# caishiqing/voice-tts

Hardware: AMD Instinct MI355X
Metric: audio_seconds_per_second (higher is better)
Workload: dtype bf16

## Files before the change

voice-tts_amd/csrc/gemm_x6.hip:

```cpp
#include "common.h"

namespace ixtts {

typedef float gx_f32x16 __attribute__((ext_vector_type(16)));
typedef __bf16 gx_bf16x8 __attribute__((ext_vector_type(8)));
typedef float gx_f32x4 __attribute__((ext_vector_type(4)));
typedef unsigned int gx_u32x4 __attribute__((ext_vector_type(4)));


__global__ void gemm_x6_pack_kernel(const float* __restrict__ w, uint4* __restrict__ out, int N, int K, int Npad) {
  const long total = (long)(K / 8) * Npad;
  for (long idx = blockIdx.x * (long)blockDim.x + threadIdx.x; idx < total; idx += (long)gridDim.x * blockDim.x) {
    const int n = (int)(idx % Npad);
    const int ko = (int)(idx / Npad);
    float v[8];
#pragma unroll
    for (int e = 0; e < 8; ++e) v[e] = n < N ? w[(long)n * K + ko * 8 + e] : 0.f;
    uint4 ph, pm, pl;
    split8_bf16x3(v, ph, pm, pl);
    const int g = ko >> 1, kh = ko & 1;
    uint4* base = out + ((long)g * 6) * Npad + n;
    base[(long)(0 * 2 + kh) * Npad] = ph;
    base[(long)(1 * 2 + kh) * Npad] = pm;
    base[(long)(2 * 2 + kh) * Npad] = pl;
  }
}

__global__ __launch_bounds__(256) void gemm_x6_split_kernel(const float* __restrict__ a, long lda, uint4* __restrict__ out, int M, int K, long Mpad) {
  __shared__ float tile[64][65];
  const int r0 = blockIdx.x * 64, k0 = blockIdx.y * 64;
  const int t = threadIdx.x;
#pragma unroll
  for (int i = 0; i < 4; ++i) {
    const int r = (t >> 4) + 16 * i, kq = t & 15;
    float4 v = make_float4(0.f, 0.f, 0.f, 0.f);
    if (r0 + r < M) v = *reinterpret_cast<const float4*>(a + (long)(r0 + r) * lda + k0 + 4 * kq);
    tile[r][4 * kq + 0] = v.x; tile[r][4 * kq + 1] = v.y; tile[r][4 * kq + 2] = v.z; tile[r][4 * kq + 3] = v.w;
  }
  __syncthreads();
#pragma unroll
  for (int u = 0; u < 2; ++u) {
    const int r = t & 63, o = (t >> 6) + 4 * u;
    float v[8];
#pragma unroll
    for (int e = 0; e < 8; ++e) v[e] = tile[r][o * 8 + e];
    uint4 ph, pm, pl;
    split8_bf16x3(v, ph, pm, pl);
    const int ko = (k0 >> 3) + o, g = ko >> 1, kh = ko & 1;
    uint4* base = out + ((long)g * 6) * Mpad + r0 + r;
    base[(long)(0 * 2 + kh) * Mpad] = ph;
    base[(long)(1 * 2 + kh) * Mpad] = pm;
    base[(long)(2 * 2 + kh) * Mpad] = pl;
  }
}

enum { EPI_PLAIN = 0, EPI_SWIGLU = 1, EPI_GATE = 2 };

struct GemmX6Params {
  const uint4* Ap;
  long Mpad;
  long arow0;
  const uint4* Wp;
  const float* bias;
  float* C;
  long ldc;
  int M, N, Npad, K, accumulate, m_tiles, n_tiles;
  int tap_steps;
  int epi;
  const float* gate;
  long gate_ld, rows_per_batch;
  int nbatch;
  const int* gate_seq_off;
  unsigned long long* dbg;
};


template <int MT, int NT, int NST, int EPI = EPI_PLAIN, int ACC = 0, int SEQ = 0, int DBG = 0, int PIN = 0>
__global__ __launch_bounds__(256, (NST * (MT + NT) * 6 * 64 * 16 <= 80 * 1024) ? 2 : 1) void gemm_x6_kernel(GemmX6Params p) {
  constexpr int BM = 64 * MT, BN = 64 * NT;
  constexpr int A_UNITS = 6 * BM, W_UNITS = 6 * BN, STAGE = A_UNITS + W_UNITS;
  constexpr int NDMA = (6 * (MT + NT)) / 4;
  constexpr int NA = (6 * MT) / 4, NW = NDMA - NA;
  static_assert((6 * MT) % 4 == 0 && (6 * NT) % 4 == 0, "the A pieces and the W pieces are each dealt evenly to the 4 waves");
  static_assert(EPI == EPI_PLAIN || (ACC == 0 && NT == 2), "pair epilogues: the wave's two 32-column blocks are the two halves");
  static_assert(EPI == EPI_GATE || SEQ == 0, "the sequence table belongs to the gate epilogue");
  constexpr int D = NST - 1;
  extern __shared__ uint4 smem[];

  const int nwg = p.m_tiles * p.n_tiles;
  const int bid = blockIdx.x;
  const int xcd = bid & 7, idx = bid >> 3;
  const int qd = nwg >> 3, rm = nwg & 7;
  const int lin = (xcd < rm ? xcd * (qd + 1) : rm * (qd + 1) + (xcd - rm) * qd) + idx;
  const int m_tile = lin / p.n_tiles, n_tile = lin - m_tile * p.n_tiles;
  const int m0 = m_tile * BM, n0 = n_tile * BN;

  const int tid = threadIdx.x, lane = tid & 63;
  const int wave = __builtin_amdgcn_readfirstlane(tid >> 6);
  const int wm = wave >> 1, wn = wave & 1;
  const int l31 = lane & 31, lh = lane >> 5;

  gx_f32x16 acc[MT][NT];
#pragma unroll
  for (int i = 0; i < MT; ++i)
#pragma unroll
    for (int j = 0; j < NT; ++j)
#pragma unroll
      for (int r = 0; r < 16; ++r) acc[i][j][r] = 0.f;

  const uint4* asrc = p.Ap + p.arow0 + m0 + lane;
  const uint4* wsrc = p.Wp + n0 + lane;
  long a_off[NA], w_off[NW];
  int a_lds[NA], w_lds[NW];
#pragma unroll
  for (int q = 0; q < NA; ++q) {
    const int e = q * 4 + wave, run = e / MT, piece = e % MT;
    a_off[q] = run * p.Mpad + piece * 64;
    a_lds[q] = run * BM + piece * 64;
  }
#pragma unroll
  for (int q = 0; q < NW; ++q) {
    const int e = q * 4 + wave, run = e / NT, piece = e % NT;
    w_off[q] = (long)run * p.Npad + piece * 64;
    w_lds[q] = A_UNITS + run * BN + piece * 64;
  }
  const long a_step = 6 * p.Mpad, w_step = 6L * p.Npad;
  const long a_wrap = 1 - p.tap_steps * a_step;
  long a_run = 0, w_run = 0;
  int a_group = 0;
  auto issue_next = [&](uint4* st) {
#pragma unroll
    for (int q = 0; q < NA; ++q)
      __builtin_amdgcn_global_load_lds((const __attribute__((address_space(1))) void*)(asrc + (a_off[q] + a_run)),
                                       (__attribute__((address_space(3))) void*)(st + a_lds[q]), 16, 0, 0);
#pragma unroll
    for (int q = 0; q < NW; ++q)
      __builtin_amdgcn_global_load_lds((const __attribute__((address_space(1))) void*)(wsrc + (w_off[q] + w_run)),
                                       (__attribute__((address_space(3))) void*)(st + w_lds[q]), 16, 0, 0);
    a_run += a_step;
    w_run += w_step;
    if (++a_group == p.tap_steps) {
      a_group = 0;
      a_run += a_wrap;
    }
  };

  const int steps = p.K >> 4;
  auto wg_stamp = [&](int k) {
    if constexpr (DBG == 3) {
      if (tid == 0) p.dbg[128 + (long)blockIdx.x * 4 + k] = __builtin_amdgcn_s_memrealtime();
    }
  };
  auto wait_younger = [&](int y) {
    if (y >= 2) asm volatile("s_waitcnt vmcnt(%0)" ::"n"(2 * NDMA) : "memory");
    else if (y == 1) asm volatile("s_waitcnt vmcnt(%0)" ::"n"(NDMA) : "memory");
    else asm volatile("s_waitcnt vmcnt(0)" ::: "memory");
  };
  static_assert(D >= 1 && D <= 3, "1..3 steps of copies in flight behind the one waited for");
  wg_stamp(0);
  for (int t = 0; t < D && t < steps; ++t) issue_next(smem + t * STAGE);
  wait_younger(min(D, steps) - 1);
  __builtin_amdgcn_s_barrier();
  asm volatile("" ::: "memory");
  wg_stamp(1);

  const unsigned base_addr = (unsigned)(uintptr_t)(const __attribute__((address_space(3))) void*)smem;
  int st_cur = 0, st_nxt = D % NST;
  for (int s = 0; s < steps; ++s) {
    auto stamp = [&](int k) {
      if constexpr (DBG == 3) {
        if (blockIdx.x == 0 && tid == 0 && s < 16) {
          p.dbg[s * 8 + k] = __builtin_amdgcn_s_memtime();
          if (k == 0) p.dbg[s * 8 + 7] = __builtin_amdgcn_s_memrealtime();
        }
      }
    };
    stamp(0);
    if (DBG != 1 && s + D < steps) issue_next(smem + st_nxt * STAGE);
    stamp(1);
    const unsigned cur_addr = base_addr + (unsigned)(st_cur * STAGE * 16);
    if constexpr (DBG != 2) {
      gx_u32x4 af[3][MT], bf[3][NT];
      const unsigned aaddr = cur_addr + (unsigned)((lh * BM + wm * (32 * MT) + l31) * 16);
      const unsigned waddr = cur_addr + (unsigned)((A_UNITS + lh * BN + wn * (32 * NT) + l31) * 16);
      if constexpr (MT == 4 && NT == 2) {
        asm volatile(
            "ds_read_b128 %0, %18 offset:%20\n ds_read_b128 %1, %18 offset:%21\n ds_read_b128 %2, %18 offset:%22\n ds_read_b128 %3, %18 offset:%23\n"
            "ds_read_b128 %4, %18 offset:%24\n ds_read_b128 %5, %18 offset:%25\n ds_read_b128 %6, %18 offset:%26\n ds_read_b128 %7, %18 offset:%27\n"
            "ds_read_b128 %8, %18 offset:%28\n ds_read_b128 %9, %18 offset:%29\n ds_read_b128 %10, %18 offset:%30\n ds_read_b128 %11, %18 offset:%31\n"
            "ds_read_b128 %12, %19 offset:%32\n ds_read_b128 %13, %19 offset:%33\n ds_read_b128 %14, %19 offset:%34\n ds_read_b128 %15, %19 offset:%35\n"
            "ds_read_b128 %16, %19 offset:%36\n ds_read_b128 %17, %19 offset:%37\n s_waitcnt lgkmcnt(0)"
            : "=&v"(af[0][0]), "=&v"(af[0][1]), "=&v"(af[0][2]), "=&v"(af[0][3]), "=&v"(af[1][0]), "=&v"(af[1][1]), "=&v"(af[1][2]), "=&v"(af[1][3]),
              "=&v"(af[2][0]), "=&v"(af[2][1]), "=&v"(af[2][2]), "=&v"(af[2][3]), "=&v"(bf[0][0]), "=&v"(bf[0][1]), "=&v"(bf[1][0]), "=&v"(bf[1][1]),
              "=&v"(bf[2][0]), "=&v"(bf[2][1])
            : "v"(aaddr), "v"(waddr), "n"((0 * 2 * BM + 0) * 16), "n"((0 * 2 * BM + 32) * 16), "n"((0 * 2 * BM + 64) * 16), "n"((0 * 2 * BM + 96) * 16),
              "n"((1 * 2 * BM + 0) * 16), "n"((1 * 2 * BM + 32) * 16), "n"((1 * 2 * BM + 64) * 16), "n"((1 * 2 * BM + 96) * 16), "n"((2 * 2 * BM + 0) * 16),
              "n"((2 * 2 * BM + 32) * 16), "n"((2 * 2 * BM + 64) * 16), "n"((2 * 2 * BM + 96) * 16), "n"((0 * 2 * BN + 0) * 16), "n"((0 * 2 * BN + 32) * 16),
              "n"((1 * 2 * BN + 0) * 16), "n"((1 * 2 * BN + 32) * 16), "n"((2 * 2 * BN + 0) * 16), "n"((2 * 2 * BN + 32) * 16)
            : "memory");
      } else {
        static_assert(MT == 2 && NT == 2, "fragment block written for 256 x 128 and 128 x 128 tiles");
        asm volatile(
            "ds_read_b128 %0, %12 offset:%14\n ds_read_b128 %1, %12 offset:%15\n ds_read_b128 %2, %12 offset:%16\n ds_read_b128 %3, %12 offset:%17\n"
            "ds_read_b128 %4, %12 offset:%18\n ds_read_b128 %5, %12 offset:%19\n ds_read_b128 %6, %13 offset:%20\n ds_read_b128 %7, %13 offset:%21\n"
            "ds_read_b128 %8, %13 offset:%22\n ds_read_b128 %9, %13 offset:%23\n ds_read_b128 %10, %13 offset:%24\n ds_read_b128 %11, %13 offset:%25\n"
            "s_waitcnt lgkmcnt(0)"
            : "=&v"(af[0][0]), "=&v"(af[0][1]), "=&v"(af[1][0]), "=&v"(af[1][1]), "=&v"(af[2][0]), "=&v"(af[2][1]), "=&v"(bf[0][0]), "=&v"(bf[0][1]),
              "=&v"(bf[1][0]), "=&v"(bf[1][1]), "=&v"(bf[2][0]), "=&v"(bf[2][1])
            : "v"(aaddr), "v"(waddr), "n"((0 * 2 * BM + 0) * 16), "n"((0 * 2 * BM + 32) * 16), "n"((1 * 2 * BM + 0) * 16), "n"((1 * 2 * BM + 32) * 16),
              "n"((2 * 2 * BM + 0) * 16), "n"((2 * 2 * BM + 32) * 16), "n"((0 * 2 * BN + 0) * 16), "n"((0 * 2 * BN + 32) * 16), "n"((1 * 2 * BN + 0) * 16),
              "n"((1 * 2 * BN + 32) * 16), "n"((2 * 2 * BN + 0) * 16), "n"((2 * 2 * BN + 32) * 16)
            : "memory");
      }
      stamp(2);
#pragma unroll
      for (int i = 0; i < MT; ++i)
#pragma unroll
        for (int j = 0; j < NT; ++j) {
          const gx_bf16x8 ah = __builtin_bit_cast(gx_bf16x8, af[0][i]), am = __builtin_bit_cast(gx_bf16x8, af[1][i]), al = __builtin_bit_cast(gx_bf16x8, af[2][i]);
          const gx_bf16x8 bh = __builtin_bit_cast(gx_bf16x8, bf[0][j]), bm = __builtin_bit_cast(gx_bf16x8, bf[1][j]), bl = __builtin_bit_cast(gx_bf16x8, bf[2][j]);
          acc[i][j] = __builtin_amdgcn_mfma_f32_32x32x16_bf16(al, bh, acc[i][j], 0, 0, 0);
          acc[i][j] = __builtin_amdgcn_mfma_f32_32x32x16_bf16(ah, bl, acc[i][j], 0, 0, 0);
          acc[i][j] = __builtin_amdgcn_mfma_f32_32x32x16_bf16(am, bm, acc[i][j], 0, 0, 0);
          acc[i][j] = __builtin_amdgcn_mfma_f32_32x32x16_bf16(am, bh, acc[i][j], 0, 0, 0);
          acc[i][j] = __builtin_amdgcn_mfma_f32_32x32x16_bf16(ah, bm, acc[i][j], 0, 0, 0);
          acc[i][j] = __builtin_amdgcn_mfma_f32_32x32x16_bf16(ah, bh, acc[i][j], 0, 0, 0);
        }
      if constexpr (DBG == 3) asm volatile("" ::"v"(acc[0][0][0]), "v"(acc[MT - 1][NT - 1][15]));
      if constexpr (PIN != 0) __builtin_amdgcn_sched_barrier(0);
    }
    stamp(3);
    wait_younger(DBG == 1 ? 0 : max(0, min(D - 1, steps - s - 2)));
    stamp(4);
    __builtin_amdgcn_s_barrier();
    asm volatile("" ::: "memory");
    stamp(5);
    st_cur = st_cur + 1 == NST ? 0 : st_cur + 1;
    st_nxt = st_nxt + 1 == NST ? 0 : st_nxt + 1;
  }

  wg_stamp(2);
  if constexpr (EPI != EPI_PLAIN) {
    const int oc = (n0 + wn * 64) / 2 + l31;
    const int nh = p.N >> 1;
    if (oc < nh) {
      const unsigned rpb = (unsigned)min(p.rows_per_batch, (long)0x7fffffff);
      const float ba = p.bias != nullptr ? p.bias[n0 + wn * 64 + l31] : 0.f, bb = p.bias != nullptr ? p.bias[n0 + wn * 64 + 32 + l31] : 0.f;
#pragma unroll
      for (int i = 0; i < MT; ++i) {
        const int rbase = m0 + wm * (32 * MT) + i * 32 + 4 * lh;
#pragma unroll
        for (int r = 0; r < 16; ++r) {
          const int row = rbase + (r & 3) + 8 * (r >> 2);
          if (row < p.M) {
            float a = acc[i][0][r] + ba, b = acc[i][1][r] + bb, v;
            if constexpr (EPI == EPI_SWIGLU) {
              v = a / (1.0f + expf(-a)) * b;
            } else {
              long gb;
              if constexpr (SEQ != 0) gb = (long)seq_of_row(p.gate_seq_off, p.nbatch, row);
              else gb = min((long)((unsigned)row / rpb), (long)p.nbatch - 1);
              const float* g = p.gate + gb * p.gate_ld;
              a += g[oc];
              b += g[nh + oc];
              v = tanhf(a) * (1.0f / (1.0f + expf(-b)));
            }
            p.C[(long)row * p.ldc + oc] = v;
          }
        }
      }
    }
  } else
#pragma unroll
  for (int j = 0; j < NT; ++j) {
    const int col = n0 + wn * (32 * NT) + j * 32 + l31;
    const bool col_ok = col < p.N;
    const float bv = (p.bias != nullptr && col_ok) ? p.bias[col] : 0.f;
#pragma unroll
    for (int i = 0; i < MT; ++i) {
      const int rbase = m0 + wm * (32 * MT) + i * 32 + 4 * lh;
#pragma unroll
      for (int r = 0; r < 16; ++r) {
        const int row = rbase + (r & 3) + 8 * (r >> 2);
        if (col_ok && row < p.M) {
          float* c = p.C + (long)row * p.ldc + col;
          float v = acc[i][j][r] + bv;
          if constexpr (ACC != 0) v += *c;
          *c = v;
        }
      }
    }
  }
  if constexpr (DBG == 3) {
    asm volatile("s_waitcnt vmcnt(0)" ::: "memory");
    wg_stamp(3);
  }
}

template <int MT, int NT, int NST, int EPI = EPI_PLAIN, int ACC = 0, int SEQ = 0, int DBG = 0, int PIN = 0>
static int launch_gemm_x6(GemmX6Params p, hipStream_t st) {
  constexpr int BM = 64 * MT, BN = 64 * NT;
  constexpr size_t smem = (size_t)NST * (6 * BM + 6 * BN) * 16;
  static_assert(smem <= 160 * 1024, "LDS stages of this tile shape");
  p.m_tiles = ceil_div(p.M, BM);
  p.n_tiles = ceil_div(p.N, BN);
  IX_ARG((long)p.n_tiles * BN <= p.Npad, "gemm_x6: packed weights padded to %d features, the %d-wide tile needs %d", p.Npad, BN, p.n_tiles * BN);
  const int taps = (p.K >> 4) / p.tap_steps;
  IX_ARG(p.arow0 + (long)p.m_tiles * BM + taps - 1 <= p.Mpad, "gemm_x6: activation planes hold %ld rows, the %d-row tiles reach row %ld", p.Mpad, BM,
         p.arow0 + (long)p.m_tiles * BM + taps - 1);
  auto kern = gemm_x6_kernel<MT, NT, NST, EPI, ACC, SEQ, DBG, PIN>;
  static bool done = false;
  if (!done) {
    IX_HIP(hipFuncSetAttribute((const void*)kern, hipFuncAttributeMaxDynamicSharedMemorySize, (int)smem));
    done = true;
  }
  hipLaunchKernelGGL(kern, dim3(p.m_tiles * p.n_tiles), dim3(256), smem, st, p);
  IX_HIP(hipGetLastError());
  return IXTTS_OK;
}

template <int MT, int NT, int NST, bool PAIR>
static int launch_gemm_x6_epilogue(const GemmX6Params& p, hipStream_t st) {
  if (p.epi == EPI_PLAIN) return p.accumulate ? launch_gemm_x6<MT, NT, NST, EPI_PLAIN, 1>(p, st) : launch_gemm_x6<MT, NT, NST, EPI_PLAIN, 0>(p, st);
  if constexpr (PAIR) {
    if (p.epi == EPI_SWIGLU) return launch_gemm_x6<MT, NT, NST, EPI_SWIGLU>(p, st);
    if (p.epi == EPI_GATE)
      return p.gate_seq_off ? launch_gemm_x6<MT, NT, NST, EPI_GATE, 0, 1>(p, st) : launch_gemm_x6<MT, NT, NST, EPI_GATE, 0, 0>(p, st);
  }
  set_error("gemm_x6: epilogue %d on a tile shape built without it", p.epi);
  return IXTTS_ERR_ARG;
}

}

using namespace ixtts;

extern "C" size_t ixtts_gemm_x6_packed_bytes(int N, int K) {
  if (N <= 0 || K <= 0 || K % 64) return 0;
  const size_t Npad = (size_t)(N + 255) / 256 * 256;
  return (size_t)(K / 16) * 6 * Npad * 16;
}

extern "C" int ixtts_gemm_x6_pack(const float* w_dev, void* packed_dev, int N, int K, void* stream) {
  IX_ARG(w_dev && packed_dev && N > 0 && K > 0 && K % 64 == 0, "gemm_x6_pack: bad argument (K must be a multiple of 64)");
  const int Npad = (N + 255) / 256 * 256;
  const long total = (long)(K / 8) * Npad;
  hipLaunchKernelGGL(gemm_x6_pack_kernel, dim3((unsigned)std::min<long>((total + 255) / 256, 4096)), dim3(256), 0, (hipStream_t)stream, w_dev,
                     reinterpret_cast<uint4*>(packed_dev), N, K, Npad);
  IX_HIP(hipGetLastError());
  return IXTTS_OK;
}

extern "C" long ixtts_gemm_x6_rows_padded(long rows) { return rows <= 0 ? 0 : (rows + 255) / 256 * 256 + 256; }

extern "C" int ixtts_gemm_x6_split(const float* a_dev, long lda, void* planes_dev, long rows, int K, void* stream) {
  IX_ARG(a_dev && planes_dev && rows > 0 && K > 0 && K % 64 == 0, "gemm_x6_split: bad argument (K must be a multiple of 64)");
  IX_ARG(lda >= K && lda % 4 == 0 && (reinterpret_cast<uintptr_t>(a_dev) & 15) == 0, "gemm_x6_split: rows must be 16-byte aligned (lda %ld)", lda);
  const long Mpad = ixtts_gemm_x6_rows_padded(rows);
  hipLaunchKernelGGL(gemm_x6_split_kernel, dim3((unsigned)(Mpad / 64), K / 64), dim3(256), 0, (hipStream_t)stream, a_dev, lda,
                     reinterpret_cast<uint4*>(planes_dev), (int)rows, K, Mpad);
  IX_HIP(hipGetLastError());
  return IXTTS_OK;
}

static int run_gemm_x6(GemmX6Params p, int tile, hipStream_t st) {
  if (tile == 0) {
    const long t42 = (long)ceil_div(p.M, 256) * ceil_div(p.N, 128);
    tile = t42 >= 140 ? 2 : 3;
  }
  switch (tile) {
    case 2: return launch_gemm_x6_epilogue<4, 2, 2, true>(p, st);
    case 3: return launch_gemm_x6_epilogue<2, 2, 3, true>(p, st);
    case 4: return launch_gemm_x6_epilogue<4, 2, 4, false>(p, st);
    case 5: return launch_gemm_x6_epilogue<2, 2, 4, false>(p, st);
  }
  if (tile >= 12 && (p.epi != EPI_PLAIN || p.accumulate)) {
    set_error("gemm_x6: the developer variants (tile %d) are built with the plain, overwriting epilogue only", tile);
    return IXTTS_ERR_ARG;
  }
  switch (tile) {
    case 12: return launch_gemm_x6<4, 2, 2, EPI_PLAIN, 0, 0, 1>(p, st);
    case 22: return launch_gemm_x6<4, 2, 2, EPI_PLAIN, 0, 0, 2>(p, st);
    case 32: return launch_gemm_x6<4, 2, 2, EPI_PLAIN, 0, 0, 3>(p, st);
    case 33: return launch_gemm_x6<2, 2, 3, EPI_PLAIN, 0, 0, 3>(p, st);
    case 42: return launch_gemm_x6<4, 2, 2, EPI_PLAIN, 0, 0, 0, 1>(p, st);
    case 43: return launch_gemm_x6<2, 2, 3, EPI_PLAIN, 0, 0, 0, 1>(p, st);
  }
  set_error("gemm_x6: tile %d (0 auto; 2 / 3: 256x128 / 128x128, two workgroups per CU; 4 / 5: the same, one per CU with a 4-stage ring)", tile);
  return IXTTS_ERR_ARG;
}

extern "C" int ixtts_gemm_x6_f32(const void* a_planes_dev, long rows_total, long row0, const void* packed_dev, const float* bias_dev, float* c_dev,
                                 long ldc, int M, int N, int K, int accumulate, int tile, void* stream) {
  IX_ARG(a_planes_dev && packed_dev && c_dev && M > 0 && N > 0 && K > 0 && K % 64 == 0, "gemm_x6: bad argument (K must be a multiple of 64: the split pass works on 64-wide k blocks)");
  IX_ARG(ldc >= N && row0 >= 0 && row0 + M <= rows_total, "gemm_x6: rows [%ld, %ld) of %ld, ldc %ld", row0, row0 + M, rows_total, ldc);
  GemmX6Params p;
  p.Ap = reinterpret_cast<const uint4*>(a_planes_dev); p.Mpad = ixtts_gemm_x6_rows_padded(rows_total); p.arow0 = row0;
  p.Wp = reinterpret_cast<const uint4*>(packed_dev); p.bias = bias_dev; p.C = c_dev; p.ldc = ldc;
  p.M = M; p.N = N; p.Npad = (N + 255) / 256 * 256; p.K = K; p.accumulate = accumulate ? 1 : 0; p.m_tiles = p.n_tiles = 0;
  p.tap_steps = K >> 4; p.epi = EPI_PLAIN; p.gate = nullptr; p.gate_ld = 0; p.rows_per_batch = 1; p.nbatch = 1; p.gate_seq_off = nullptr;
  p.dbg = (tile == 32 || tile == 33) ? reinterpret_cast<unsigned long long*>(const_cast<float*>(bias_dev)) : nullptr;
  if (p.dbg) p.bias = nullptr;
  return run_gemm_x6(p, tile, (hipStream_t)stream);
}

extern "C" int ixtts_gemm_x6_pair_f32(const void* a_planes_dev, long rows_total, long row0, int taps, const void* packed_dev, const float* bias_dev,
                                      const float* gate_dev, long gate_ld, long rows_per_batch, int nbatch, float* c_dev, long ldc, int M, int N, int K,
                                      int epilogue, int tile, void* stream) {
  IX_ARG(a_planes_dev && packed_dev && c_dev && M > 0 && N > 0 && taps > 0 && K > 0, "gemm_x6_pair: bad argument");
  IX_ARG(K % taps == 0 && (K / taps) % 64 == 0 && N % 64 == 0, "gemm_x6_pair: K %d = %d taps of a multiple of 64, N %d a multiple of 64", K, taps, N);
  IX_ARG(epilogue == EPI_SWIGLU || (epilogue == EPI_GATE && gate_dev && rows_per_batch > 0 && nbatch > 0 && gate_ld >= N / 2),
         "gemm_x6_pair: epilogue %d (1 swiglu; 2 gate, with gate biases)", epilogue);
  IX_ARG(ldc >= N / 2 && row0 >= 0 && row0 + M + taps - 1 <= rows_total, "gemm_x6_pair: rows [%ld, %ld) + %d taps of %ld, ldc %ld", row0, row0 + M, taps,
         rows_total, ldc);
  IX_ARG(tile == 0 || tile == 2 || tile == 3, "gemm_x6_pair: tile %d (0 auto, 2, 3)", tile);
  GemmX6Params p;
  p.Ap = reinterpret_cast<const uint4*>(a_planes_dev); p.Mpad = ixtts_gemm_x6_rows_padded(rows_total); p.arow0 = row0;
  p.Wp = reinterpret_cast<const uint4*>(packed_dev); p.bias = bias_dev; p.C = c_dev; p.ldc = ldc;
  p.M = M; p.N = N; p.Npad = (N + 255) / 256 * 256; p.K = K; p.accumulate = 0; p.m_tiles = p.n_tiles = 0;
  p.tap_steps = (K / taps) >> 4; p.epi = epilogue; p.gate = gate_dev; p.gate_ld = gate_ld; p.rows_per_batch = rows_per_batch; p.nbatch = nbatch;
  p.gate_seq_off = nullptr;
  p.dbg = nullptr;
  return run_gemm_x6(p, tile, (hipStream_t)stream);
}

extern "C" int ixtts_gemm_x6_pair_gate_varlen_f32(const void* a_planes_dev, long rows_total, long row0, int taps, const void* packed_dev, const float* bias_dev,
                                                  const float* gate_dev, long gate_ld, const int* seq_off_dev, int nseq, float* c_dev, long ldc, int M, int N,
                                                  int K, int tile, void* stream) {
  IX_ARG(seq_off_dev && nseq > 0, "gemm_x6_pair_gate_varlen: null offsets table or nseq %d", nseq);
  IX_ARG(a_planes_dev && packed_dev && c_dev && gate_dev && M > 0 && N > 0 && taps > 0 && K > 0 && gate_ld >= N / 2, "gemm_x6_pair_gate_varlen: bad argument");
  IX_ARG(K % taps == 0 && (K / taps) % 64 == 0 && N % 64 == 0, "gemm_x6_pair_gate_varlen: K %d = %d taps of a multiple of 64, N %d a multiple of 64", K, taps, N);
  IX_ARG(ldc >= N / 2 && row0 >= 0 && row0 + M + taps - 1 <= rows_total, "gemm_x6_pair_gate_varlen: rows [%ld, %ld) + %d taps of %ld, ldc %ld", row0, row0 + M,
         taps, rows_total, ldc);
  IX_ARG(tile == 0 || tile == 2 || tile == 3, "gemm_x6_pair_gate_varlen: tile %d (0 auto, 2, 3)", tile);
  GemmX6Params p;
  p.Ap = reinterpret_cast<const uint4*>(a_planes_dev); p.Mpad = ixtts_gemm_x6_rows_padded(rows_total); p.arow0 = row0;
  p.Wp = reinterpret_cast<const uint4*>(packed_dev); p.bias = bias_dev; p.C = c_dev; p.ldc = ldc;
  p.M = M; p.N = N; p.Npad = (N + 255) / 256 * 256; p.K = K; p.accumulate = 0; p.m_tiles = p.n_tiles = 0;
  p.tap_steps = (K / taps) >> 4; p.epi = EPI_GATE; p.gate = gate_dev; p.gate_ld = gate_ld; p.rows_per_batch = 1; p.nbatch = nseq;
  p.gate_seq_off = seq_off_dev;
  p.dbg = nullptr;
  return run_gemm_x6(p, tile, (hipStream_t)stream);
}
```

Measured before the change: 41.86.

## Add software-pipelined 128x128 GEMM loop with interleaved MFMA and LDS reads

Adds a PIPE variant of the x6 bf16 GEMM kernel (128x128 tile, 4-stage ring, one workgroup per CU). Its main loop double-buffers register fragments and uses inline asm to interleave ds_read_b128 for the next step with the MFMAs of the current step. Global-to-LDS copies are split into pieces spread between the MFMA quarters. The auto tile selector now uses this variant for mid-sized grids with K of at least 1024, trading occupancy and added hand-scheduled asm complexity for hiding LDS and DMA latency.

```diff
diff --git a/voice-tts_amd/csrc/gemm_x6.hip b/voice-tts_amd/csrc/gemm_x6.hip
--- a/voice-tts_amd/csrc/gemm_x6.hip
+++ b/voice-tts_amd/csrc/gemm_x6.hip
@@ -75,7 +75,33 @@
 };
 
 
-template <int MT, int NT, int NST, int EPI = EPI_PLAIN, int ACC = 0, int SEQ = 0, int DBG = 0, int PIN = 0>
+#define GX6_MFMA(c, a, b) "v_mfma_f32_32x32x16_bf16 %" #c ", %" #a ", %" #b ", %" #c "\n"
+#define GX6_READ(n, o) "ds_read_b128 %" #n ", %14 offset:%" #o "\n"
+#define GX6_QUARTER(...)                                                                                                                        \
+  asm volatile(__VA_ARGS__                                                                                                                      \
+               : "+v"(c0), "+v"(c1), "=&v"(n0), "=&v"(n1), "=&v"(n2)                                                                            \
+               : "v"(ah), "v"(am), "v"(al), "v"(bh0), "v"(bm0), "v"(bl0), "v"(bh1), "v"(bm1), "v"(bl1), "v"(addr), "n"(O0), "n"(O1), "n"(O2)  \
+               : "memory")
+template <int HALF, int READ, int O0, int O1, int O2>
+__device__ __forceinline__ void gemm_x6_pipe_quarter(gx_f32x16& c0, gx_f32x16& c1, const gx_u32x4& ah, const gx_u32x4& am, const gx_u32x4& al,
+                                                     const gx_u32x4& bh0, const gx_u32x4& bm0, const gx_u32x4& bl0, const gx_u32x4& bh1,
+                                                     const gx_u32x4& bm1, const gx_u32x4& bl1, gx_u32x4& n0, gx_u32x4& n1, gx_u32x4& n2, unsigned addr) {
+  if constexpr (HALF == 0 && READ != 0)
+    GX6_QUARTER(GX6_MFMA(0, 7, 8) GX6_READ(2, 15) GX6_READ(3, 16) GX6_MFMA(1, 7, 11) GX6_READ(4, 17) GX6_MFMA(0, 5, 10) GX6_MFMA(1, 5, 13)
+                GX6_MFMA(0, 6, 9) GX6_MFMA(1, 6, 12) "s_waitcnt lgkmcnt(0)");
+  else if constexpr (HALF == 0)
+    GX6_QUARTER(GX6_MFMA(0, 7, 8) GX6_MFMA(1, 7, 11) GX6_MFMA(0, 5, 10) GX6_MFMA(1, 5, 13) GX6_MFMA(0, 6, 9) GX6_MFMA(1, 6, 12));
+  else if constexpr (READ != 0)
+    GX6_QUARTER(GX6_MFMA(0, 6, 8) GX6_READ(2, 15) GX6_READ(3, 16) GX6_MFMA(1, 6, 11) GX6_READ(4, 17) GX6_MFMA(0, 5, 9) GX6_MFMA(1, 5, 12)
+                GX6_MFMA(0, 5, 8) GX6_MFMA(1, 5, 11) "s_waitcnt lgkmcnt(0)");
+  else
+    GX6_QUARTER(GX6_MFMA(0, 6, 8) GX6_MFMA(1, 6, 11) GX6_MFMA(0, 5, 9) GX6_MFMA(1, 5, 12) GX6_MFMA(0, 5, 8) GX6_MFMA(1, 5, 11));
+}
+#undef GX6_QUARTER
+#undef GX6_READ
+#undef GX6_MFMA
+
+template <int MT, int NT, int NST, int EPI = EPI_PLAIN, int ACC = 0, int SEQ = 0, int DBG = 0, int PIN = 0, int PIPE = 0>
 __global__ __launch_bounds__(256, (NST * (MT + NT) * 6 * 64 * 16 <= 80 * 1024) ? 2 : 1) void gemm_x6_kernel(GemmX6Params p) {
   constexpr int BM = 64 * MT, BN = 64 * NT;
   constexpr int A_UNITS = 6 * BM, W_UNITS = 6 * BN, STAGE = A_UNITS + W_UNITS;
@@ -84,6 +110,7 @@
   static_assert((6 * MT) % 4 == 0 && (6 * NT) % 4 == 0, "the A pieces and the W pieces are each dealt evenly to the 4 waves");
   static_assert(EPI == EPI_PLAIN || (ACC == 0 && NT == 2), "pair epilogues: the wave's two 32-column blocks are the two halves");
   static_assert(EPI == EPI_GATE || SEQ == 0, "the sequence table belongs to the gate epilogue");
+  static_assert(PIPE == 0 || (MT == 2 && NT == 2 && NST == 4), "pipelined loop: 128 x 128 tile, 4 stages");
   constexpr int D = NST - 1;
   extern __shared__ uint4 smem[];
 
@@ -159,13 +186,108 @@
   static_assert(D >= 1 && D <= 3, "1..3 steps of copies in flight behind the one waited for");
   wg_stamp(0);
   for (int t = 0; t < D && t < steps; ++t) issue_next(smem + t * STAGE);
-  wait_younger(min(D, steps) - 1);
+  wait_younger(PIPE != 0 ? D - 2 : min(D, steps) - 1);
   __builtin_amdgcn_s_barrier();
   asm volatile("" ::: "memory");
   wg_stamp(1);
 
   const unsigned base_addr = (unsigned)(uintptr_t)(const __attribute__((address_space(3))) void*)smem;
+
+  if constexpr (PIPE != 0) {
+    gx_u32x4 fa[2][3][MT], fb[2][3][NT];
+    const unsigned a_lane = (unsigned)((lh * BM + wm * (32 * MT) + l31) * 16), w_lane = (unsigned)((A_UNITS + lh * BN + wn * (32 * NT) + l31) * 16);
+    int st_rd = 1, st_is = D % NST;
+    auto issue_pieces = [&](uint4* st, int q0, int q1) {
+#pragma unroll
+      for (int q = 0; q < NA; ++q)
+        if (q >= q0 && q < q1)
+          __builtin_amdgcn_global_load_lds((const __attribute__((address_space(1))) void*)(asrc + (a_off[q] + a_run)),
+                                           (__attribute__((address_space(3))) void*)(st + a_lds[q]), 16, 0, 0);
+#pragma unroll
+      for (int q = 0; q < NW; ++q)
+        if (NA + q >= q0 && NA + q < q1)
+          __builtin_amdgcn_global_load_lds((const __attribute__((address_space(1))) void*)(wsrc + (w_off[q] + w_run)),
+                                           (__attribute__((address_space(3))) void*)(st + w_lds[q]), 16, 0, 0);
+      if (q1 != NDMA) return;
+      a_run += a_step;
+      w_run += w_step;
+      if (++a_group == p.tap_steps) {
+        a_group = 0;
+        a_run += a_wrap;
+      }
+    };
+    auto pipe_step = [&](auto mode, int s, gx_u32x4 (&ca)[3][MT], gx_u32x4 (&cb)[3][NT], gx_u32x4 (&na)[3][MT], gx_u32x4 (&nb)[3][NT]) {
+      constexpr int MODE = decltype(mode)::value, RD = MODE != 0;
+      auto stamp = [&](int k) {
+        if constexpr (DBG == 3) {
+          if (blockIdx.x == 0 && tid == 0 && s < 16) {
+            p.dbg[s * 8 + k] = __builtin_amdgcn_s_memtime();
+            if (k == 0) p.dbg[s * 8 + 7] = __builtin_amdgcn_s_memrealtime();
+          }
+        }
+      };
+      stamp(0);
+      const bool more = DBG != 1 && (MODE == 2 || (MODE == 1 && s + D < steps));
+      uint4* ist = smem + st_is * STAGE;
+      const unsigned aaddr = base_addr + (unsigned)(st_rd * STAGE * 16) + a_lane, waddr = base_addr + (unsigned)(st_rd * STAGE * 16) + w_lane;
+      constexpr int PA = 2 * BM * 16, PW = 2 * BN * 16;
+      gemm_x6_pipe_quarter<0, RD, 0, PA, 2 * PA>(acc[0][0], acc[0][1], ca[0][0], ca[1][0], ca[2][0], cb[0][0], cb[1][0], cb[2][0], cb[0][1], cb[1][1],
+                                                 cb[2][1], na[0][0], na[1][0], na[2][0], aaddr);
+      if (more) issue_pieces(ist, 0, 2);
+      stamp(1);
+      gemm_x6_pipe_quarter<1, RD, 512, PA + 512, 2 * PA + 512>(acc[0][0], acc[0][1], ca[0][0], ca[1][0], ca[2][0], cb[0][0], cb[1][0], cb[2][0], cb[0][1],
+                                                               cb[1][1], cb[2][1], na[0][1], na[1][1], na[2][1], aaddr);
+      if (more) issue_pieces(ist, 2, 4);
+      stamp(2);
+      gemm_x6_pipe_quarter<0, RD, 0, PW, 2 * PW>(acc[1][0], acc[1][1], ca[0][1], ca[1][1], ca[2][1], cb[0][0], cb[1][0], cb[2][0], cb[0][1], cb[1][1],
+                                                 cb[2][1], nb[0][0], nb[1][0], nb[2][0], waddr);
+      if (more) issue_pieces(ist, 4, NDMA);
+      gemm_x6_pipe_quarter<1, RD, 512, PW + 512, 2 * PW + 512>(acc[1][0], acc[1][1], ca[0][1], ca[1][1], ca[2][1], cb[0][0], cb[1][0], cb[2][0], cb[0][1],
+                                                               cb[1][1], cb[2][1], nb[0][1], nb[1][1], nb[2][1], waddr);
+      stamp(3);
+      if constexpr (MODE == 0) return;
+      if constexpr (MODE == 2 && DBG != 1) wait_younger(D - 2);
+      else wait_younger(DBG == 1 ? 0 : max(0, min(D - 2, steps - s - 3)));
+      stamp(4);
+      __builtin_amdgcn_s_barrier();
+      asm volatile("" ::: "memory");
+      stamp(5);
+      st_rd = st_rd + 1 == NST ? 0 : st_rd + 1;
+      st_is = st_is + 1 == NST ? 0 : st_is + 1;
+    };
+    const std::integral_constant<int, 2> steady;
+    const std::integral_constant<int, 1> tail;
+    const std::integral_constant<int, 0> last;
+    {
+      gx_u32x4 (&af)[3][MT] = fa[0], (&bf)[3][NT] = fb[0];
+      const unsigned aaddr = base_addr + a_lane, waddr = base_addr + w_lane;
+      asm volatile(
+          "ds_read_b128 %0, %12 offset:%14\n ds_read_b128 %1, %12 offset:%15\n ds_read_b128 %2, %12 offset:%16\n ds_read_b128 %3, %12 offset:%17\n"
+          "ds_read_b128 %4, %12 offset:%18\n ds_read_b128 %5, %12 offset:%19\n ds_read_b128 %6, %13 offset:%20\n ds_read_b128 %7, %13 offset:%21\n"
+          "ds_read_b128 %8, %13 offset:%22\n ds_read_b128 %9, %13 offset:%23\n ds_read_b128 %10, %13 offset:%24\n ds_read_b128 %11, %13 offset:%25\n"
+          "s_waitcnt lgkmcnt(0)"
+          : "=&v"(af[0][0]), "=&v"(af[0][1]), "=&v"(af[1][0]), "=&v"(af[1][1]), "=&v"(af[2][0]), "=&v"(af[2][1]), "=&v"(bf[0][0]), "=&v"(bf[0][1]),
+            "=&v"(bf[1][0]), "=&v"(bf[1][1]), "=&v"(bf[2][0]), "=&v"(bf[2][1])
+          : "v"(aaddr), "v"(waddr), "n"((0 * 2 * BM + 0) * 16), "n"((0 * 2 * BM + 32) * 16), "n"((1 * 2 * BM + 0) * 16), "n"((1 * 2 * BM + 32) * 16),
+            "n"((2 * 2 * BM + 0) * 16), "n"((2 * 2 * BM + 32) * 16), "n"((0 * 2 * BN + 0) * 16), "n"((0 * 2 * BN + 32) * 16), "n"((1 * 2 * BN + 0) * 16),
+            "n"((1 * 2 * BN + 32) * 16), "n"((2 * 2 * BN + 0) * 16), "n"((2 * 2 * BN + 32) * 16)
+          : "memory");
+    }
+    int s = 0;
+    for (; s + 1 + D < steps; s += 2) {
+      pipe_step(steady, s, fa[0], fb[0], fa[1], fb[1]);
+      pipe_step(steady, s + 1, fa[1], fb[1], fa[0], fb[0]);
+    }
+    for (; s < steps - 2; s += 2) {
+      pipe_step(tail, s, fa[0], fb[0], fa[1], fb[1]);
+      pipe_step(tail, s + 1, fa[1], fb[1], fa[0], fb[0]);
+    }
+    pipe_step(tail, steps - 2, fa[0], fb[0], fa[1], fb[1]);
+    pipe_step(last, steps - 1, fa[1], fb[1], fa[0], fb[0]);
+    asm volatile("s_nop 15" : "+v"(acc[0][0]), "+v"(acc[0][1]), "+v"(acc[1][0]), "+v"(acc[1][1]));
+  }
   int st_cur = 0, st_nxt = D % NST;
+  if constexpr (PIPE == 0)
   for (int s = 0; s < steps; ++s) {
     auto stamp = [&](int k) {
       if constexpr (DBG == 3) {
@@ -297,7 +419,7 @@
   }
 }
 
-template <int MT, int NT, int NST, int EPI = EPI_PLAIN, int ACC = 0, int SEQ = 0, int DBG = 0, int PIN = 0>
+template <int MT, int NT, int NST, int EPI = EPI_PLAIN, int ACC = 0, int SEQ = 0, int DBG = 0, int PIN = 0, int PIPE = 0>
 static int launch_gemm_x6(GemmX6Params p, hipStream_t st) {
   constexpr int BM = 64 * MT, BN = 64 * NT;
   constexpr size_t smem = (size_t)NST * (6 * BM + 6 * BN) * 16;
@@ -308,7 +430,7 @@
   const int taps = (p.K >> 4) / p.tap_steps;
   IX_ARG(p.arow0 + (long)p.m_tiles * BM + taps - 1 <= p.Mpad, "gemm_x6: activation planes hold %ld rows, the %d-row tiles reach row %ld", p.Mpad, BM,
          p.arow0 + (long)p.m_tiles * BM + taps - 1);
-  auto kern = gemm_x6_kernel<MT, NT, NST, EPI, ACC, SEQ, DBG, PIN>;
+  auto kern = gemm_x6_kernel<MT, NT, NST, EPI, ACC, SEQ, DBG, PIN, PIPE>;
   static bool done = false;
   if (!done) {
     IX_HIP(hipFuncSetAttribute((const void*)kern, hipFuncAttributeMaxDynamicSharedMemorySize, (int)smem));
@@ -319,13 +441,14 @@
   return IXTTS_OK;
 }
 
-template <int MT, int NT, int NST, bool PAIR>
+template <int MT, int NT, int NST, bool PAIR, int PIPE = 0>
 static int launch_gemm_x6_epilogue(const GemmX6Params& p, hipStream_t st) {
-  if (p.epi == EPI_PLAIN) return p.accumulate ? launch_gemm_x6<MT, NT, NST, EPI_PLAIN, 1>(p, st) : launch_gemm_x6<MT, NT, NST, EPI_PLAIN, 0>(p, st);
+  if (p.epi == EPI_PLAIN)
+    return p.accumulate ? launch_gemm_x6<MT, NT, NST, EPI_PLAIN, 1, 0, 0, 0, PIPE>(p, st) : launch_gemm_x6<MT, NT, NST, EPI_PLAIN, 0, 0, 0, 0, PIPE>(p, st);
   if constexpr (PAIR) {
-    if (p.epi == EPI_SWIGLU) return launch_gemm_x6<MT, NT, NST, EPI_SWIGLU>(p, st);
+    if (p.epi == EPI_SWIGLU) return launch_gemm_x6<MT, NT, NST, EPI_SWIGLU, 0, 0, 0, 0, PIPE>(p, st);
     if (p.epi == EPI_GATE)
-      return p.gate_seq_off ? launch_gemm_x6<MT, NT, NST, EPI_GATE, 0, 1>(p, st) : launch_gemm_x6<MT, NT, NST, EPI_GATE, 0, 0>(p, st);
+      return p.gate_seq_off ? launch_gemm_x6<MT, NT, NST, EPI_GATE, 0, 1, 0, 0, PIPE>(p, st) : launch_gemm_x6<MT, NT, NST, EPI_GATE, 0, 0, 0, 0, PIPE>(p, st);
   }
   set_error("gemm_x6: epilogue %d on a tile shape built without it", p.epi);
   return IXTTS_ERR_ARG;
@@ -367,12 +490,14 @@
   if (tile == 0) {
     const long t42 = (long)ceil_div(p.M, 256) * ceil_div(p.N, 128);
     tile = t42 >= 140 ? 2 : 3;
+    if (tile == 3 && (long)ceil_div(p.M, 128) * ceil_div(p.N, 128) <= 256 && p.K >= 1024) tile = 6;
   }
   switch (tile) {
     case 2: return launch_gemm_x6_epilogue<4, 2, 2, true>(p, st);
     case 3: return launch_gemm_x6_epilogue<2, 2, 3, true>(p, st);
     case 4: return launch_gemm_x6_epilogue<4, 2, 4, false>(p, st);
     case 5: return launch_gemm_x6_epilogue<2, 2, 4, false>(p, st);
+    case 6: return launch_gemm_x6_epilogue<2, 2, 4, true, 1>(p, st);
   }
   if (tile >= 12 && (p.epi != EPI_PLAIN || p.accumulate)) {
     set_error("gemm_x6: the developer variants (tile %d) are built with the plain, overwriting epilogue only", tile);
@@ -380,13 +505,15 @@
   }
   switch (tile) {
     case 12: return launch_gemm_x6<4, 2, 2, EPI_PLAIN, 0, 0, 1>(p, st);
+    case 16: return launch_gemm_x6<2, 2, 4, EPI_PLAIN, 0, 0, 1, 0, 1>(p, st);
     case 22: return launch_gemm_x6<4, 2, 2, EPI_PLAIN, 0, 0, 2>(p, st);
     case 32: return launch_gemm_x6<4, 2, 2, EPI_PLAIN, 0, 0, 3>(p, st);
     case 33: return launch_gemm_x6<2, 2, 3, EPI_PLAIN, 0, 0, 3>(p, st);
+    case 36: return launch_gemm_x6<2, 2, 4, EPI_PLAIN, 0, 0, 3, 0, 1>(p, st);
     case 42: return launch_gemm_x6<4, 2, 2, EPI_PLAIN, 0, 0, 0, 1>(p, st);
     case 43: return launch_gemm_x6<2, 2, 3, EPI_PLAIN, 0, 0, 0, 1>(p, st);
   }
-  set_error("gemm_x6: tile %d (0 auto; 2 / 3: 256x128 / 128x128, two workgroups per CU; 4 / 5: the same, one per CU with a 4-stage ring)", tile);
+  set_error("gemm_x6: tile %d (0 auto; 2 / 3: 256x128 / 128x128, two workgroups per CU; 4 / 5: the same, one per CU with a 4-stage ring; 6: 128x128, one per CU, pipelined loop)", tile);
   return IXTTS_ERR_ARG;
 }
 
@@ -399,7 +526,7 @@
   p.Wp = reinterpret_cast<const uint4*>(packed_dev); p.bias = bias_dev; p.C = c_dev; p.ldc = ldc;
   p.M = M; p.N = N; p.Npad = (N + 255) / 256 * 256; p.K = K; p.accumulate = accumulate ? 1 : 0; p.m_tiles = p.n_tiles = 0;
   p.tap_steps = K >> 4; p.epi = EPI_PLAIN; p.gate = nullptr; p.gate_ld = 0; p.rows_per_batch = 1; p.nbatch = 1; p.gate_seq_off = nullptr;
-  p.dbg = (tile == 32 || tile == 33) ? reinterpret_cast<unsigned long long*>(const_cast<float*>(bias_dev)) : nullptr;
+  p.dbg = (tile == 32 || tile == 33 || tile == 36) ? reinterpret_cast<unsigned long long*>(const_cast<float*>(bias_dev)) : nullptr;
   if (p.dbg) p.bias = nullptr;
   return run_gemm_x6(p, tile, (hipStream_t)stream);
 }
@@ -413,7 +540,7 @@
          "gemm_x6_pair: epilogue %d (1 swiglu; 2 gate, with gate biases)", epilogue);
   IX_ARG(ldc >= N / 2 && row0 >= 0 && row0 + M + taps - 1 <= rows_total, "gemm_x6_pair: rows [%ld, %ld) + %d taps of %ld, ldc %ld", row0, row0 + M, taps,
          rows_total, ldc);
-  IX_ARG(tile == 0 || tile == 2 || tile == 3, "gemm_x6_pair: tile %d (0 auto, 2, 3)", tile);
+  IX_ARG(tile == 0 || tile == 2 || tile == 3 || tile == 6, "gemm_x6_pair: tile %d (0 auto, 2, 3, 6)", tile);
   GemmX6Params p;
   p.Ap = reinterpret_cast<const uint4*>(a_planes_dev); p.Mpad = ixtts_gemm_x6_rows_padded(rows_total); p.arow0 = row0;
   p.Wp = reinterpret_cast<const uint4*>(packed_dev); p.bias = bias_dev; p.C = c_dev; p.ldc = ldc;
@@ -432,7 +559,7 @@
   IX_ARG(K % taps == 0 && (K / taps) % 64 == 0 && N % 64 == 0, "gemm_x6_pair_gate_varlen: K %d = %d taps of a multiple of 64, N %d a multiple of 64", K, taps, N);
   IX_ARG(ldc >= N / 2 && row0 >= 0 && row0 + M + taps - 1 <= rows_total, "gemm_x6_pair_gate_varlen: rows [%ld, %ld) + %d taps of %ld, ldc %ld", row0, row0 + M,
          taps, rows_total, ldc);
-  IX_ARG(tile == 0 || tile == 2 || tile == 3, "gemm_x6_pair_gate_varlen: tile %d (0 auto, 2, 3)", tile);
+  IX_ARG(tile == 0 || tile == 2 || tile == 3 || tile == 6, "gemm_x6_pair_gate_varlen: tile %d (0 auto, 2, 3, 6)", tile);
   GemmX6Params p;
   p.Ap = reinterpret_cast<const uint4*>(a_planes_dev); p.Mpad = ixtts_gemm_x6_rows_padded(rows_total); p.arow0 = row0;
   p.Wp = reinterpret_cast<const uint4*>(packed_dev); p.bias = bias_dev; p.C = c_dev; p.ldc = ldc;
```

Measured after the change: 42.11, median of 6. Within noise of the previous version (+0.6%).
